# lopunch/CWBNWP-LETKF

Hardware: AMD Instinct MI355X
Metric: analysis grid-points/sec (+ wall-clock per cycle) at k=40, 1/2/4/8 MI355X (higher is better)
Workload: dtype f64

## Files before the change

cwbnwp-letkf_amd/csrc/cwbl_tq40_fill.hip:

```cpp
#include "cwbl_tq40_common.h"

#include <utility>

namespace cwbl {

namespace {

__device__ __forceinline__ void rsum16x2(double &a, double &b) {
  double ab[2] = {a, b};
  rsum16xN(ab);
  a = ab[0];
  b = ab[1];
}

__device__ __forceinline__ void touch(double &x) { asm volatile("" : "+v"(x)); }
__device__ __forceinline__ int touched(int x) {
  asm volatile("" : "+v"(x));
  return x;
}
__device__ __forceinline__ long long touched(long long x) {
  asm volatile("" : "+v"(x));
  return x;
}

template <int KP>
__device__ __forceinline__ void tq40_factor_solve(
    const SolveConsts &c, const SlabDev &slab, Tq40Smem<KP> &sm,
    double (&A)[Tq40Layout<KP>::NS][KP], const long long g0, const bool valid, const int ptot, const int gi, const int q, const int l,
    int2 *__restrict__ info) {
  using LY = Tq40Layout<KP>;
  constexpr int J0 = LY::J0, KT = LY::KT, NS = LY::NS, NV = LY::NV, H = LY::H;
  using SM = Tq40Smem<KP>;
  const int k = c.k;
  const int lp = l < J0 ? l : 0;
  const bool pre = l < J0;
  auto vrow = [&](int vs) { return tq40_vrow<KP>(l, vs); };
  int *const pkeep = reinterpret_cast<int *>(&sm.tq[q][KP][3]);
  *pkeep = ptot;
  const double trace = tq40_trace(sm, q, l, k);

  const double m = (double)c.inflat;
  const double ratio = trace / m - (double)(k - 1);
  int level = 1;
  double dec = 10.0;
  while (level < kQuadLevels && dec < ratio) {
    dec *= 10.0;
    ++level;
  }
  const int R = tq40_wave_rounds(level);
  const int NQ = 8 * R - 1;
  const double2 *qtab = quad_rule(c.quad_r, R, level);
  const int side = l >> 3, n8 = l & 7;
  const double(*T)[4] = sm.tq[q];
  char *const smb = reinterpret_cast<char *>(&sm);
  auto lds = [&](unsigned off) { return *reinterpret_cast<const double *>(smb + off); };
  auto sts = [&](unsigned off, double v) { *reinterpret_cast<double *>(smb + off) = v; };
  const unsigned tq0 = (unsigned)(offsetof(SM, tq) + (size_t)q * sizeof(sm.tq[0])) +
                       (side ? (KP - 1) * 32u : 0u);
  const unsigned dirb = side ? (unsigned)-32 : 32u;
  const unsigned csb = side ? 40u : 8u;
  const unsigned qs0 = (unsigned)(offsetof(SM, qs) + (size_t)q * sizeof(sm.qs[0])) +
                       (side ? (KP - H) * 8u : (H - 1) * 8u);
  const unsigned qz0 = (unsigned)(offsetof(SM, qz) + (size_t)q * sizeof(sm.qz[0]));
  const unsigned bdir = side ? 8u : (unsigned)-8;
  const double sk = sqrt((double)(k - 1));
  auto touch_cols = [&]() {
    sfor<KT - 2>([&](auto jj) {
      constexpr int jl = decltype(jj)::value, J1 = jl + 1, R1 = J1 / 16;
      sfor<NS>([&](auto rr) {
        constexpr int r = decltype(rr)::value;
        if constexpr (16 * r + 15 > J1 || r == R1) touch(A[r][J0 + jl]);
      });
    });
  };

  float *__restrict__ const var = slab.var;
  const int use_rtpp = c.use_rtpp, use_rtps = c.use_rtps;
  const float rtpp_alpha = c.rtpp_alpha, rtps_alpha = c.rtps_alpha;

  float xbl[NV];
  double xb_mean;
  {
    const long long P = tq40_var_index(slab, g0, valid ? gi : 0);
    sfor<NV>([&](auto vv) {
      constexpr int vs = decltype(vv)::value;
      const int i = vrow(vs);
      const bool mem = valid && i < k;
      const float xv = var[P + slab.L * (mem ? i : 0)];
      xbl[vs] = mem ? xv : 0.0f;
    });
    xb_mean = (double)(seq_sum_f32<KP>(xbl) * c.nmember_inv);
  }
  double uxP = pre && l < k ? (double)xbl[0] - xb_mean : 0.0, ux[NS];
  sfor<NS>([&](auto rr) {
    constexpr int r = decltype(rr)::value;
    const int t = J0 + l + 16 * r;
    ux[r] = t < k ? (double)xbl[r + 1] - xb_mean : 0.0;
  });

  touch_cols();
  sfor<J0>([&](auto jj) {
    constexpr int j = decltype(jj)::value, J1 = j + 1;
    const double *pj = sm.pv[q][j];
    const double scal = pj[0], tau = sm.tau[q][j];
    double u2a;
    if constexpr (J1 < J0) u2a = rbcast<J1>(uxP);
    else u2a = rbcast<0>(ux[0]);
    const double xP = (pre && l > J1) ? pj[lp] : 0.0;
    double x[NS], xu = xP * uxP;
    sfor<NS>([&](auto rr) {
      constexpr int r = decltype(rr)::value;
      x[r] = pj[J0 + l + 16 * r];
      xu = fma(x[r], ux[r], xu);
    });
    xu = rsum16(xu);
    const double xsP = xP * scal;
    const double vP = (pre && l == J1) ? 1.0 : xsP;
    const double s2 = fma(scal, xu, u2a);
    uxP = fma(-tau * s2, vP, uxP);
    sfor<NS>([&](auto rr) {
      constexpr int r = decltype(rr)::value;
      const double xs = x[r] * scal;
      double vr;
      if constexpr (J1 == J0 && r == 0) vr = l == 0 ? 1.0 : xs;
      else vr = xs;
      ux[r] = fma(-tau * s2, vr, ux[r]);
    });
  });
  sfor<KT - 2>([&](auto jj) {
    constexpr int jl = decltype(jj)::value, j = J0 + jl;
    constexpr int J1 = jl + 1, R1 = J1 / 16, L1 = J1 % 16;
    const double scal = rbcast<L1>(A[R1][j]), tau = sm.tau[q][j];
    double x[NS], xu = 0.0;
    sfor<NS>([&](auto rr) {
      constexpr int r = decltype(rr)::value;
      if constexpr (16 * r + 15 > J1) {
        const int t = l + 16 * r;
        if constexpr (r == R1) x[r] = t == J1 ? 0.0 : A[r][j];
        else x[r] = A[r][j];
        xu = fma(x[r], ux[r], xu);
      } else {
        x[r] = 0.0;
      }
    });
    xu = rsum16(xu);
    const double s2 = fma(scal, xu, rbcast<L1>(ux[R1]));
    sfor<NS>([&](auto rr) {
      constexpr int r = decltype(rr)::value;
      const int t = l + 16 * r;
      const double xs = x[r] * scal;
      const double vr = t == J1 ? 1.0 : xs;
      ux[r] = fma(-tau * s2, vr, ux[r]);
    });
  });
  if (pre) sm.tq[q][l][3] = uxP;
  sfor<NS>([&](auto rr) {
    constexpr int r = decltype(rr)::value;
    sm.tq[q][J0 + l + 16 * r][3] = ux[r];
  });
  __syncthreads();

  double ys[NV], z[NV];
  sfor<NV>([&](auto vv) { ys[decltype(vv)::value] = 0.0; });
  for (int round = 0; round < R; ++round) {
    const int node = 8 * round + n8;
    const double2 tw = qtab[min(node, NQ - 1)];
    const double sigma = node < NQ ? m * tw.x : 0.0;
    const double omega = node < NQ ? sqrt(m) * tw.y : 1.0;
    double hh[H], mm[H];
    unsigned pw = tq0;
    double dl = lds(pw) + sigma, gt = lds(pw + 24);
    double rdl = rcp64(dl);
    sfor<H - 1>([&](auto tt) {
      constexpr int t = decltype(tt)::value + 1;
      pw += dirb;
      asm volatile("" : "+v"(pw) : "v"(dl));
      const double ct = lds(pw + csb);
      const double lt = ct * rdl;
      hh[t - 1] = gt * rdl;
      mm[t - 1] = lt;
      dl = fma(-lt, ct, lds(pw) + sigma);
      gt = fma(-lt, gt, lds(pw + 24));
      rdl = rcp64(dl);
    });
    const double cm = T[H][1];
    const double dlo = ror8(dl), go = ror8(gt);
    double xv = (gt * dlo - cm * go) / fma(dl, dlo, -cm * cm);
    const bool last = round == R - 1;
    const bool zlane = last && n8 == 7;
    const double om = zlane ? 0.0 : omega;
    unsigned ps = qs0;
    unsigned pz = qz0 + (zlane ? qs0 - (unsigned)offsetof(SM, qs) - (unsigned)q * KP * 8u
                               : KP * 8u);
    const unsigned zdir = zlane ? bdir : 0u;
    auto emit = [&](double x) {
      double s = om * x;
      s += dpp_f64<0xB1>(s);
      s += dpp_f64<0x4E>(s);
      s += dpp_f64<0x141>(s);
      sts(ps, s);
      sts(pz, x);
    };
    emit(xv);
    sfor<H - 1>([&](auto tt) {
      constexpr int t = H - 2 - decltype(tt)::value;
      xv = fma(-mm[t], xv, hh[t]);
      ps += bdir;
      pz += zdir;
      asm volatile("" : "+v"(ps), "+v"(pz) : "v"(xv));
      emit(xv);
    });
    __syncthreads();
    sfor<NV>([&](auto vv) {
      constexpr int vs = decltype(vv)::value;
      const int i = vrow(vs);
      const int ic = i < KP ? i : 0;
      ys[vs] += i < KP ? sm.qs[q][ic] : 0.0;
      if (last) z[vs] = i < KP ? sm.qz[q][ic] : 0.0;
    });
    __syncthreads();
  }
  double dpart = 0.0;
  sfor<NV>([&](auto vv) {
    constexpr int vs = decltype(vv)::value;
    const int i = vrow(vs);
    const double u1 = sm.tq[q][i < KP ? i : 0][2];
    dpart = i < KP ? fma(u1, z[vs], dpart) : dpart;
  });
  const double d = rsum16(dpart);

  double y[NV];
  sfor<NV>([&](auto vv) { y[decltype(vv)::value] = ys[decltype(vv)::value]; });
  touch_cols();
  const int lb = touched(l);
  sfor<KT - 2>([&](auto jj) {
    constexpr int jl = KT - 3 - decltype(jj)::value, j = J0 + jl, J1 = jl + 1;
    constexpr int R1 = J1 / 16, L1 = J1 % 16;
    const double tj = sm.tau[q][j];
    const double scal = rbcast<L1>(A[R1][j]);
    double vv[NS], a = 0.0;
    sfor<NS>([&](auto rr) {
      constexpr int r = decltype(rr)::value;
      if constexpr (16 * r + 15 >= J1) {
        const int t = lb + 16 * r;
        if constexpr (16 * r + 15 > J1) vv[r] = t == J1 ? 1.0 : A[r][j] * scal;
        else vv[r] = t == J1 ? 1.0 : 0.0;
        a = fma(vv[r], y[r + 1], a);
      } else {
        vv[r] = 0.0;
      }
    });
    a = rsum16(a);
    sfor<NS>([&](auto rr) {
      constexpr int r = decltype(rr)::value;
      if constexpr (16 * r + 15 >= J1) y[r + 1] = fma(-tj * a, vv[r], y[r + 1]);
    });
  });
  sfor<J0>([&](auto jj) {
    constexpr int j = J0 - 1 - decltype(jj)::value, J1 = j + 1;
    const double tj = sm.tau[q][j];
    const double *pj = sm.pv[q][j];
    const double scal = pj[0];
    const double v0 = lb == J1 ? 1.0 : (lb < J0 && lb > J1) ? pj[lb] * scal : 0.0;
    double vv[NS];
    double a = v0 * y[0];
    sfor<NS>([&](auto rr) {
      constexpr int r = decltype(rr)::value;
      const double pr = pj[J0 + lb + 16 * r] * scal;
      if constexpr (J1 == J0 && r == 0) vv[r] = lb == 0 ? 1.0 : pr;
      else vv[r] = pr;
      a = fma(vv[r], y[r + 1], a);
    });
    a = rsum16(a);
    y[0] = fma(-tj * a, v0, y[0]);
    sfor<NS>([&](auto rr) {
      constexpr int r = decltype(rr)::value;
      y[r + 1] = fma(-tj * a, vv[r], y[r + 1]);
    });
  });

  float xa[NV];
  sfor<NV>([&](auto vv) {
    constexpr int vs = decltype(vv)::value;
    xa[vs] = vrow(vs) < k ? (float)(xb_mean + (d + sk * y[vs])) : 0.0f;
  });
  if (use_rtpp || use_rtps) {
    const float xa_mean = seq_sum_f32<KP>(xa) * c.nmember_inv;
    double xpl[NV];
    float xap[NV];
    sfor<NV>([&](auto vv) {
      constexpr int vs = decltype(vv)::value;
      const bool mem = vrow(vs) < k;
      xpl[vs] = mem ? (double)xbl[vs] - xb_mean : 0.0;
      xap[vs] = 0.0f;
      if (mem) {
        xap[vs] = xa[vs] - xa_mean;
        if (use_rtpp)
          xap[vs] = (float)((double)((1.0f - rtpp_alpha) * xap[vs]) +
                            (double)rtpp_alpha * xpl[vs]);
      }
    });
    if (use_rtps) {
      double d8 = 0.0;
      sfor<KP>([&](auto mm) {
        constexpr int mb = decltype(mm)::value;
        constexpr int vs = mb < J0 ? 0 : 1 + (mb - J0) / 16, ln = mb < J0 ? mb : (mb - J0) % 16;
        const double xp = rbcast<ln>(xpl[vs]);
        d8 = d8 + xp * xp;
      });
      const float xb_std = (float)d8;
      float sq[NV];
      sfor<NV>([&](auto vv) {
        constexpr int vs = decltype(vv)::value;
        sq[vs] = xap[vs] * xap[vs];
      });
      const float xa_std = seq_sum_f32<KP>(sq);
      const float f = rtps_alpha * sqrtf(xb_std / xa_std) - rtps_alpha + 1.0f;
      sfor<NV>([&](auto vv) { xap[decltype(vv)::value] = xap[decltype(vv)::value] * f; });
    }
    sfor<NV>([&](auto vv) { xa[decltype(vv)::value] = xa_mean + xap[decltype(vv)::value]; });
  }
  const int pt = *pkeep;
  if (valid && pt > 0) {
    const long long P = tq40_var_index(slab, g0, touched(gi));
    sfor<NV>([&](auto vv) {
      constexpr int vs = decltype(vv)::value;
      const int i = vrow(vs);
      if (i < k) var[P + slab.L * i] = xa[vs];
    });
    if (l == 0) info[gi] = make_int2(pt, ratio > dec ? -level : level);
  }
}

}

template <int KP>
__global__ void __launch_bounds__(64, 2)
fill_tq40_factor_kernel(SolveConsts c, SlabDev slab, long long g0, int npts,
                        double *__restrict__ ws, double *__restrict__ aux,
                        int2 *__restrict__ info) {
  using LY = Tq40Layout<KP>;
  using FR = FactorRecord<KP>;
  using FA = FactorAux<KP>;
  constexpr int J0 = LY::J0, KT = LY::KT, NS = LY::NS;
  using SM = Tq40Smem<KP>;
  __shared__ SM sm;

  const int lane = threadIdx.x, q = lane >> 4, l = lane & 15;
  const int g4 = xcd_remap_rev(blockIdx.x, gridDim.x);
  const int gi = 4 * g4 + q;
  const bool valid = gi < npts;
  const int k = c.k;
  const int ptot = valid ? info[gi].x : 0;

  double A[NS][KP];
  double Pb[J0];
  const bool pre = l < J0;
  double ubP, ub[NS];
  tq40_load_record<KP>(ws, g4, q, l, valid, npts, A, Pb, ubP, ub);

  sfor<J0>([&](auto jj) {
    constexpr int j = decltype(jj)::value, J1 = j + 1;
    const double dj = rbcast<j>(Pb[j]);
    double alpha, u1a;
    if constexpr (J1 < J0) {
      alpha = rbcast<J1>(Pb[j]);
      u1a = rbcast<J1>(ubP);
    } else {
      alpha = rbcast<0>(A[0][j]);
      u1a = rbcast<0>(ub[0]);
    }
    const double xP = (pre && l > J1 && l < k) ? Pb[j] : 0.0;
    double x[NS];
    double xx = xP * xP, xb = xP * ubP;
    sfor<NS>([&](auto rr) {
      constexpr int r = decltype(rr)::value;
      const int i = J0 + l + 16 * r;
      x[r] = (i > J1 && i < k) ? A[r][j] : 0.0;
      xx = fma(x[r], x[r], xx);
      xb = fma(x[r], ub[r], xb);
    });
    rsum16x2(xx, xb);
    auto src_of = [&](auto cc, const double &vp, const double (&vs)[NS]) -> const double & {
      constexpr int col = decltype(cc)::value;
      if constexpr (col < J0) return vp;
      else return vs[(col - J0) / 16];
    };
    auto lane_of = [](int col) { return col < J0 ? col : (col - J0) % 16; };
    const Refl h = dlarfg(alpha, xx);
    sm.tq[q][j][0] = dj;
    sm.tq[q][J1][1] = h.beta;
    sm.tau[q][j] = h.tau;
    const double tau = h.tau;
    const double xsP = xP * h.scal;
    double vP = (pre && l == J1) ? 1.0 : xsP;
    double v[NS];
    sm.pv[q][j][(pre && l > 1) ? l : 1] = xP;
    sfor<NS>([&](auto rr) {
      constexpr int r = decltype(rr)::value;
      const double xs = x[r] * h.scal;
      if constexpr (J1 == J0 && r == 0) v[r] = l == 0 ? 1.0 : xs;
      else v[r] = xs;
      sm.pv[q][j][J0 + l + 16 * r] = x[r];
    });
    sm.pv[q][j][0] = h.scal;
    const double s3 = fma(h.scal, xb, u1a);
    ubP = fma(-tau * s3, vP, ubP);
    sfor<NS>([&](auto rr) {
      constexpr int r = decltype(rr)::value;
      ub[r] = fma(-tau * s3, v[r], ub[r]);
    });
    dpp_pin(vP);
    sfor<NS>([&](auto rr) { dpp_pin(v[decltype(rr)::value]); });
    double pa[kNA][NS], pP = 0.0;
    sfor<kNA * NS>([&](auto ii) { pa[decltype(ii)::value / NS][decltype(ii)::value % NS] = 0.0; });
    sfor<KP - J1>([&](auto cc) {
      constexpr int col = J1 + decltype(cc)::value;
      constexpr int LC = lane_of(col);
      const double &vs = src_of(std::integral_constant<int, col>{}, vP, v);
      sfor<NS>([&](auto rr) {
        constexpr int r = decltype(rr)::value;
        constexpr int a = (col - J1) % kNA;
        pa[a][r] = fmac_row<LC>(pa[a][r], vs, A[r][col]);
      });
      if constexpr (col < J0) pP = fmac_row<LC>(pP, vs, Pb[col]);
    });
    if constexpr (J1 < J0) {
      constexpr int NC = J0 - J1, CH = 3;
      sfor<(NC + CH - 1) / CH>([&](auto kk) {
        constexpr int c0 = J1 + CH * decltype(kk)::value;
        constexpr int n = J0 - c0 < CH ? J0 - c0 : CH;
        double cs[n];
        sfor<n>([&](auto cc) {
          constexpr int col = c0 + decltype(cc)::value;
          double s = 0.0;
          sfor<NS>([&](auto rr) {
            constexpr int r = decltype(rr)::value;
            s = fma(A[r][col], v[r], s);
          });
          cs[decltype(cc)::value] = s;
        });
        rsum16xN(cs);
        sfor<n>([&](auto cc) {
          constexpr int col = c0 + decltype(cc)::value;
          pP += l == col ? cs[decltype(cc)::value] : 0.0;
        });
      });
    }
    double pp[NS];
    double sp = vP * pP;
    sfor<NS>([&](auto rr) {
      constexpr int r = decltype(rr)::value;
      pp[r] = acc_sum(pa, r);
      sp = fma(v[r], pp[r], sp);
    });
    const double s1 = tau * rsum16(sp);
    const double wP = fma(-0.5 * tau * s1, vP, tau * pP);
    double wv[NS];
    sfor<NS>([&](auto rr) {
      constexpr int r = decltype(rr)::value;
      wv[r] = fma(-0.5 * tau * s1, v[r], tau * pp[r]);
    });
    double wPp = wP;
    dpp_pin(wPp);
    sfor<NS>([&](auto rr) { dpp_pin(wv[decltype(rr)::value]); });
    sfor<(KP - J1 + kUG - 1) / kUG>([&](auto pp) {
      constexpr int c0 = J1 + kUG * decltype(pp)::value;
      sfor<2>([&](auto hh) {
        constexpr int h = decltype(hh)::value;
        sfor<kUG>([&](auto ee) {
          constexpr int col = c0 + decltype(ee)::value;
          if constexpr (col < KP) {
            constexpr int LC = lane_of(col);
            const double &vs = src_of(std::integral_constant<int, col>{}, vP, v);
            const double &ws = src_of(std::integral_constant<int, col>{}, wPp, wv);
            sfor<NS>([&](auto rr) {
              constexpr int r = decltype(rr)::value;
              if constexpr (h == 0) A[r][col] = fnmac_row<LC>(A[r][col], vs, wv[r]);
              else A[r][col] = fnmac_row<LC>(A[r][col], ws, v[r]);
            });
            if constexpr (col < J0) {
              if constexpr (h == 0) Pb[col] = fnmac_row<LC>(Pb[col], vs, wPp);
              else Pb[col] = fnmac_row<LC>(Pb[col], ws, vP);
            }
          }
        });
      });
    });
  });
  __syncthreads();
  if (pre) sm.tq[q][l][2] = ubP;

  sfor<KT>([&](auto jj) {
    constexpr int jl = decltype(jj)::value, j = J0 + jl;
    constexpr int RJ = jl / 16, LJ = jl % 16;
    const double dj = rbcast<LJ>(A[RJ][j]);
    if constexpr (jl + 2 < KT) {
      constexpr int J1 = jl + 1, R1 = J1 / 16, L1 = J1 % 16;
      const double alpha = rbcast<L1>(A[R1][j]);
      double x[NS], xx = 0.0, xb = 0.0;
      sfor<NS>([&](auto rr) {
        constexpr int r = decltype(rr)::value;
        if constexpr (16 * r + 15 > J1) {
          const int i = J0 + l + 16 * r;
          x[r] = (i > j + 1 && i < k) ? A[r][j] : 0.0;
          xx = fma(x[r], x[r], xx);
          xb = fma(x[r], ub[r], xb);
        } else {
          x[r] = 0.0;
        }
      });
      rsum16x2(xx, xb);
      const Refl h = dlarfg(alpha, xx);
      const double tau = h.tau;
      sm.tq[q][j][0] = dj;
      sm.tq[q][j + 1][1] = h.beta;
      sm.tau[q][j] = tau;
      double v[NS];
      sfor<NS>([&](auto rr) {
        constexpr int r = decltype(rr)::value;
        const int t = l + 16 * r;
        const double xs = x[r] * h.scal;
        v[r] = t == J1 ? 1.0 : xs;
        if constexpr (r == R1) A[r][j] = t == J1 ? h.scal : x[r];
        else if constexpr (16 * r + 15 > J1) A[r][j] = x[r];
      });
      const double s3 = fma(h.scal, xb, rbcast<L1>(ub[R1]));
      sfor<NS>([&](auto rr) {
        constexpr int r = decltype(rr)::value;
        ub[r] = fma(-tau * s3, v[r], ub[r]);
      });
      double pa[kNA][NS];
      sfor<kNA * NS>([&](auto ii) { pa[decltype(ii)::value / NS][decltype(ii)::value % NS] = 0.0; });
      sfor<NS>([&](auto rr) { dpp_pin(v[decltype(rr)::value]); });
      sfor<KT - J1>([&](auto cc) {
        constexpr int cl = J1 + decltype(cc)::value;
        sfor<NS>([&](auto rr) {
          constexpr int r = decltype(rr)::value;
          if constexpr (16 * r + 15 > jl) {
            constexpr int a = (cl - J1) % kNA;
            pa[a][r] = fmac_row<cl % 16>(pa[a][r], v[cl / 16], A[r][J0 + cl]);
          }
        });
      });
      double pp[NS], sp = 0.0;
      sfor<NS>([&](auto rr) {
        constexpr int r = decltype(rr)::value;
        pp[r] = acc_sum(pa, r);
        if constexpr (16 * r + 15 > jl) sp = fma(v[r], pp[r], sp);
      });
      const double s1 = tau * rsum16(sp);
      double wv[NS];
      sfor<NS>([&](auto rr) {
        constexpr int r = decltype(rr)::value;
        wv[r] = fma(-0.5 * tau * s1, v[r], tau * pp[r]);
      });
      sfor<NS>([&](auto rr) { dpp_pin(wv[decltype(rr)::value]); });
      sfor<(KT - J1 + kUG - 1) / kUG>([&](auto pp) {
        constexpr int c0 = J1 + kUG * decltype(pp)::value;
        sfor<2>([&](auto hh) {
          constexpr int h = decltype(hh)::value;
          sfor<kUG>([&](auto ee) {
            constexpr int cl = c0 + decltype(ee)::value;
            if constexpr (cl < KT) {
              sfor<NS>([&](auto rr) {
                constexpr int r = decltype(rr)::value;
                if constexpr (16 * r + 15 > jl) {
                  if constexpr (h == 0)
                    A[r][J0 + cl] = fnmac_row<cl % 16>(A[r][J0 + cl], v[cl / 16], wv[r]);
                  else
                    A[r][J0 + cl] = fnmac_row<cl % 16>(A[r][J0 + cl], wv[cl / 16], v[r]);
                }
              });
            }
          });
        });
      });
    } else {
      const double ej = rbcast<LJ>(A[RJ][j - 1]);
      sm.tq[q][j][0] = dj;
      if constexpr (jl == KT - 1) sm.tq[q][j][1] = ej;
    }
  });
  sfor<NS>([&](auto rr) {
    constexpr int r = decltype(rr)::value;
    const int i = J0 + l + 16 * r;
    sm.tq[q][i][2] = ub[r];
  });
  if (l == 0) {
    sm.tq[q][0][1] = 0.0;
    sm.tq[q][KP][1] = 0.0;
  }
  __syncthreads();

  if (valid) {
    const unsigned wb = (unsigned)gi * (unsigned)FR::WORDS;
    auto st = [&](unsigned w, double x) { gst(ws, 8u * (wb + w), x); };
    sfor<(KP + 15) / 16>([&](auto rr) {
      constexpr int r = decltype(rr)::value;
      const int i = l + 16 * r;
      if (16 * r + 15 < KP || i < KP) st((unsigned)(FR::D + i), sm.tq[q][i][0]);
    });
    if (pre) st((unsigned)(FR::U1 + l), ubP);
    sfor<NS>([&](auto rr) {
      constexpr int r = decltype(rr)::value;
      st((unsigned)(FR::U1 + J0 + l + 16 * r), ub[r]);
    });
    sfor<J0>([&](auto jj) {
      constexpr int j = decltype(jj)::value, J1 = j + 1;
      const double *pj = sm.pv[q][j];
      if (pre && l >= J1) st((unsigned)(FR::col(j) + l - J1), pj[l == J1 ? 0 : l]);
      sfor<NS>([&](auto rr) {
        constexpr int r = decltype(rr)::value;
        const int i = J0 + l + 16 * r;
        if constexpr (J1 == J0 && r == 0) st((unsigned)(FR::col(j) + i - J1), pj[l == 0 ? 0 : i]);
        else st((unsigned)(FR::col(j) + i - J1), pj[i]);
      });
    });
    sfor<KT - 2>([&](auto jj) {
      constexpr int jl = decltype(jj)::value, j = J0 + jl, J1 = jl + 1;
      sfor<NS>([&](auto rr) {
        constexpr int r = decltype(rr)::value;
        if constexpr (16 * r + 15 >= J1) {
          const int t = l + 16 * r;
          if (t >= J1) st((unsigned)(FR::col(j) + t - J1), A[r][j]);
        }
      });
    });
    if (l == 0) st((unsigned)FR::EL, 0.0);
    const unsigned ab = (unsigned)gi * (unsigned)FA::WORDS;
    sfor<(KP + 15) / 16>([&](auto rr) {
      constexpr int r = decltype(rr)::value;
      const int i = l + 16 * r;
      if (16 * r + 15 < KP || i < KP) {
        gst(aux, 8u * (ab + (unsigned)(FA::B + i)), sm.tq[q][i][1]);
        const double tj = sm.tau[q][i < KP - 2 ? i : 0];
        gst(aux, 8u * (ab + (unsigned)(FA::T + i)), i < KP - 2 ? tj : 0.0);
      }
    });
  }

  tq40_factor_solve<KP>(c, slab, sm, A, g0, valid, ptot, gi, q, l, info);
}

template <int KP>
__global__ void __launch_bounds__(64, 2)
solve_tq40_factor_kernel(SolveConsts c, SlabDev slab, long long g0, int npts,
                         const double *__restrict__ ws, const double *__restrict__ aux,
                         int2 *__restrict__ info) {
  using LY = Tq40Layout<KP>;
  using FR = FactorRecord<KP>;
  using FA = FactorAux<KP>;
  constexpr int J0 = LY::J0, KT = LY::KT, NS = LY::NS;
  using SM = Tq40Smem<KP>;
  __shared__ SM sm;

  const int lane = threadIdx.x, q = lane >> 4, l = lane & 15;
  const int g4 = xcd_remap_rev(blockIdx.x, gridDim.x);
  const int gi = 4 * g4 + q;
  const bool valid = gi < npts;
  const int ptot = valid ? info[gi].x : 0;
  const bool pre = l < J0;

  const __amdgpu_buffer_rsrc_t rs = rec_rsrc(ws + (size_t)(4 * g4) * FR::WORDS, 4 * FR::WORDS);
  const unsigned rq = (unsigned)(valid ? q : npts - 4 * g4) * (unsigned)FR::WORDS;
  auto rw = [&](unsigned vword, unsigned cword) {
    const unsigned cb = 8u * cword;
    const auto v = __builtin_amdgcn_raw_buffer_load_b64(rs, (int)(8u * vword + (cb & 4095u)),
                                                        (int)(cb & ~4095u), 0);
    return __longlong_as_double(((long long)v[1] << 32) | (unsigned)v[0]);
  };
  auto rwb = [&](unsigned vbyte, unsigned cword) {
    const unsigned cb = 8u * cword;
    const auto v = __builtin_amdgcn_raw_buffer_load_b64(rs, (int)(vbyte + (cb & 4095u)),
                                                        (int)(cb & ~4095u), 0);
    return __longlong_as_double(((long long)v[1] << 32) | (unsigned)v[0]);
  };
  const unsigned rl = rq + (unsigned)l;
  double A[NS][KP];
  double c1P[J0], c1[J0][NS];
  sfor<J0>([&](auto jj) {
    constexpr int j = decltype(jj)::value, J1 = j + 1;
    c1P[j] = rw(rq + (unsigned)((pre && l > J1) ? l - J1 : 0), (unsigned)FR::col(j));
    sfor<NS>([&](auto rr) {
      constexpr int r = decltype(rr)::value;
      if constexpr (J1 == J0 && r == 0)
        c1[j][r] = rwb(rec_off(l != 0, (int)rl), (unsigned)(FR::col(j) + J0 + 16 * r - J1));
      else
        c1[j][r] = rw(rl, (unsigned)(FR::col(j) + J0 + 16 * r - J1));
    });
  });
  sfor<KT - 2>([&](auto jj) {
    constexpr int jl = decltype(jj)::value, j = J0 + jl, J1 = jl + 1;
    sfor<NS>([&](auto rr) {
      constexpr int r = decltype(rr)::value;
      if constexpr (16 * r >= J1) {
        A[r][j] = rw(rl, (unsigned)(FR::col(j) + 16 * r - J1));
      } else if constexpr (16 * r + 15 >= J1) {
        const int t = l + 16 * r;
        A[r][j] = rwb(rec_off(t >= J1, (int)rq + t - J1), (unsigned)FR::col(j));
      }
    });
  });
  double dg[(KP + 15) / 16];
  sfor<(KP + 15) / 16>([&](auto rr) {
    constexpr int r = decltype(rr)::value;
    const int i = l + 16 * r;
    dg[r] = rw(rq + (unsigned)(i < KP ? i : 0), (unsigned)FR::D);
  });
  double ubP, ub[NS];
  {
    const double b = rw(rq + (unsigned)(pre ? l : 0), (unsigned)FR::U1);
    ubP = pre ? b : 0.0;
  }
  sfor<NS>([&](auto rr) {
    constexpr int r = decltype(rr)::value;
    ub[r] = rw(rl, (unsigned)(FR::U1 + J0 + 16 * r));
  });
  const __amdgpu_buffer_rsrc_t ra = rec_rsrc(aux + (size_t)(4 * g4) * FA::WORDS, 4 * FA::WORDS);
  const unsigned aq = (unsigned)(valid ? q : npts - 4 * g4) * (unsigned)FA::WORDS;
  constexpr int NA = (KP + 15) / 16;
  static_assert(16 * (NA - 1) + 8 == KP, "the last run of an aux half is half a row");
  const int l2 = l < 8 ? l + 16 * (NA - 1) : l + 16 * (NA - 2);
  auto arow = [&](int r) { return r < NA - 1 ? l + 16 * r : l2; };
  double bt[NA], ta[NA];
  sfor<NA>([&](auto rr) {
    constexpr int r = decltype(rr)::value;
    const unsigned off = 8u * (aq + (unsigned)arow(r));
    const auto vb = __builtin_amdgcn_raw_buffer_load_b64(ra, (int)(off + 8u * FA::B), 0, 0);
    const auto vt = __builtin_amdgcn_raw_buffer_load_b64(ra, (int)(off + 8u * FA::T), 0, 0);
    bt[r] = __longlong_as_double(((long long)vb[1] << 32) | (unsigned)vb[0]);
    ta[r] = __longlong_as_double(((long long)vt[1] << 32) | (unsigned)vt[0]);
  });

  sfor<(KP + 15) / 16>([&](auto rr) {
    constexpr int r = decltype(rr)::value;
    const int i = l + 16 * r;
    sm.tq[q][i < KP ? i : KP][0] = dg[r];
  });
  sm.tq[q][pre ? l : KP][2] = ubP;
  sfor<NS>([&](auto rr) {
    constexpr int r = decltype(rr)::value;
    sm.tq[q][J0 + l + 16 * r][2] = ub[r];
  });
  sfor<NA>([&](auto rr) {
    constexpr int r = decltype(rr)::value;
    sm.tq[q][arow(r)][1] = bt[r];
    sm.tau[q][arow(r)] = ta[r];
  });
  sm.tq[q][KP][1] = 0.0;

  sfor<J0>([&](auto jj) {
    constexpr int j = decltype(jj)::value, J1 = j + 1;
    sm.pv[q][j][(pre && l > J1) ? l : 0] = c1P[j];
    sfor<NS>([&](auto rr) {
      constexpr int r = decltype(rr)::value;
      sm.pv[q][j][J0 + l + 16 * r] = c1[j][r];
    });
  });
  __syncthreads();

  tq40_factor_solve<KP>(c, slab, sm, A, g0, valid, ptot, gi, q, l, info);
}

hipError_t launch_fill_tq40_factor(hipStream_t s, int kp, SolveConsts c, SlabDev slab,
                                   long long g0, int npts, double *ws, double *aux, int2 *info) {
  if (npts <= 0) return hipSuccess;
  if (c.quad_r == nullptr || aux == nullptr || kp != kTq4KP) return hipErrorInvalidValue;
  const dim3 grid((npts + 3) / 4);
  hipLaunchKernelGGL((fill_tq40_factor_kernel<kTq4KP>), grid, dim3(64), 0, s, c, slab, g0, npts,
                     ws, aux, info);
  return hipGetLastError();
}

hipError_t launch_solve_tq40_factor(hipStream_t s, int kp, SolveConsts c, SlabDev slab,
                                    long long g0, int npts, const double *ws, const double *aux,
                                    int2 *info) {
  if (npts <= 0) return hipSuccess;
  if (c.quad_r == nullptr || aux == nullptr || kp != kTq4KP) return hipErrorInvalidValue;
  const dim3 grid((npts + 3) / 4);
  hipLaunchKernelGGL((solve_tq40_factor_kernel<kTq4KP>), grid, dim3(64), 0, s, c, slab, g0, npts,
                     ws, aux, info);
  return hipGetLastError();
}

}
```

Measured before the change: 417.2 million.

## Prefetch background state, quadrature nodes and LDS rows ahead in TQ40 solve

Hoists the background-ensemble loads out of the factor solve so the solve kernel can issue them earlier, interleaved with the factor reloads. An AHEAD template variant prefetches the next quadrature node and the next tridiagonal row from LDS one step early, and it reorders when the register columns are touched. The RTPS spread is now computed from squares taken once per lane and reduced via DPP row ops. These changes aim to hide global and LDS latency, at the cost of higher register pressure that may lower occupancy.

```diff
diff --git a/cwbnwp-letkf_amd/csrc/cwbl_tq40_fill.hip b/cwbnwp-letkf_amd/csrc/cwbl_tq40_fill.hip
--- a/cwbnwp-letkf_amd/csrc/cwbl_tq40_fill.hip
+++ b/cwbnwp-letkf_amd/csrc/cwbl_tq40_fill.hip
@@ -24,9 +24,23 @@
 }
 
 template <int KP>
+__device__ __forceinline__ void tq40_load_xb(const SlabDev &slab, const long long g0,
+                                             const bool valid, const int gi, const int l,
+                                             const int k, float (&xv)[Tq40Layout<KP>::NV]) {
+  const float *__restrict__ const var = slab.var;
+  const long long P = tq40_var_index(slab, g0, valid ? gi : 0);
+  sfor<Tq40Layout<KP>::NV>([&](auto vv) {
+    constexpr int vs = decltype(vv)::value;
+    const int i = tq40_vrow<KP>(l, vs);
+    xv[vs] = var[P + slab.L * ((valid && i < k) ? i : 0)];
+  });
+}
+
+template <int KP, bool AHEAD>
 __device__ __forceinline__ void tq40_factor_solve(
     const SolveConsts &c, const SlabDev &slab, Tq40Smem<KP> &sm,
-    double (&A)[Tq40Layout<KP>::NS][KP], const long long g0, const bool valid, const int ptot, const int gi, const int q, const int l,
+    double (&A)[Tq40Layout<KP>::NS][KP], const float (&xbv)[Tq40Layout<KP>::NV], const long long g0,
+    const bool valid, const int ptot, const int gi, const int q, const int l,
     int2 *__restrict__ info) {
   using LY = Tq40Layout<KP>;
   constexpr int J0 = LY::J0, KT = LY::KT, NS = LY::NS, NV = LY::NV, H = LY::H;
@@ -50,6 +64,8 @@
   const int R = tq40_wave_rounds(level);
   const int NQ = 8 * R - 1;
   const double2 *qtab = quad_rule(c.quad_r, R, level);
+  double2 twn;
+  if constexpr (AHEAD) twn = qtab[min(l & 7, NQ - 1)];
   const int side = l >> 3, n8 = l & 7;
   const double(*T)[4] = sm.tq[q];
   char *const smb = reinterpret_cast<char *>(&sm);
@@ -81,13 +97,10 @@
   float xbl[NV];
   double xb_mean;
   {
-    const long long P = tq40_var_index(slab, g0, valid ? gi : 0);
     sfor<NV>([&](auto vv) {
       constexpr int vs = decltype(vv)::value;
-      const int i = vrow(vs);
-      const bool mem = valid && i < k;
-      const float xv = var[P + slab.L * (mem ? i : 0)];
-      xbl[vs] = mem ? xv : 0.0f;
+      const bool mem = valid && vrow(vs) < k;
+      xbl[vs] = mem ? xbv[vs] : 0.0f;
     });
     xb_mean = (double)(seq_sum_f32<KP>(xbl) * c.nmember_inv);
   }
@@ -98,7 +111,6 @@
     ux[r] = t < k ? (double)xbl[r + 1] - xb_mean : 0.0;
   });
 
-  touch_cols();
   sfor<J0>([&](auto jj) {
     constexpr int j = decltype(jj)::value, J1 = j + 1;
     const double *pj = sm.pv[q][j];
@@ -130,6 +142,10 @@
   sfor<KT - 2>([&](auto jj) {
     constexpr int jl = decltype(jj)::value, j = J0 + jl;
     constexpr int J1 = jl + 1, R1 = J1 / 16, L1 = J1 % 16;
+    sfor<NS>([&](auto rr) {
+      constexpr int r = decltype(rr)::value;
+      if constexpr (16 * r + 15 > J1 || r == R1) touch(A[r][j]);
+    });
     const double scal = rbcast<L1>(A[R1][j]), tau = sm.tau[q][j];
     double x[NS], xu = 0.0;
     sfor<NS>([&](auto rr) {
@@ -164,24 +180,43 @@
   sfor<NV>([&](auto vv) { ys[decltype(vv)::value] = 0.0; });
   for (int round = 0; round < R; ++round) {
     const int node = 8 * round + n8;
-    const double2 tw = qtab[min(node, NQ - 1)];
+    double2 tw;
+    if constexpr (AHEAD) {
+      tw = twn;
+      if (round + 1 < R) twn = qtab[min(node + 8, NQ - 1)];
+    } else {
+      tw = qtab[min(node, NQ - 1)];
+    }
     const double sigma = node < NQ ? m * tw.x : 0.0;
     const double omega = node < NQ ? sqrt(m) * tw.y : 1.0;
     double hh[H], mm[H];
     unsigned pw = tq0;
     double dl = lds(pw) + sigma, gt = lds(pw + 24);
-    double rdl = rcp64(dl);
+    double nd, nc, ng;
+    auto next_row = [&]() {
+      pw += dirb;
+      nd = lds(pw);
+      nc = lds(pw + csb);
+      ng = lds(pw + 24);
+    };
+    if constexpr (AHEAD) next_row();
     sfor<H - 1>([&](auto tt) {
       constexpr int t = decltype(tt)::value + 1;
-      pw += dirb;
-      asm volatile("" : "+v"(pw) : "v"(dl));
-      const double ct = lds(pw + csb);
+      if constexpr (!AHEAD) {
+        asm volatile("" : "+v"(pw) : "v"(dl));
+        next_row();
+      }
+      const double dt = nd, ct = nc, g = ng;
+      if constexpr (AHEAD && t < H - 1) {
+        asm volatile("" : "+v"(pw) : "v"(dl));
+        next_row();
+      }
+      const double rdl = rcp64(dl);
       const double lt = ct * rdl;
       hh[t - 1] = gt * rdl;
       mm[t - 1] = lt;
-      dl = fma(-lt, ct, lds(pw) + sigma);
-      gt = fma(-lt, gt, lds(pw + 24));
-      rdl = rcp64(dl);
+      dl = fma(-lt, ct, dt + sigma);
+      gt = fma(-lt, gt, g);
     });
     const double cm = T[H][1];
     const double dlo = ror8(dl), go = ror8(gt);
@@ -301,12 +336,16 @@
       }
     });
     if (use_rtps) {
-      double d8 = 0.0;
+      double d8 = 0.0, sq8[NV];
+      sfor<NV>([&](auto vv) {
+        constexpr int vs = decltype(vv)::value;
+        sq8[vs] = xpl[vs] * xpl[vs];
+        dpp_pin(sq8[vs]);
+      });
       sfor<KP>([&](auto mm) {
         constexpr int mb = decltype(mm)::value;
         constexpr int vs = mb < J0 ? 0 : 1 + (mb - J0) / 16, ln = mb < J0 ? mb : (mb - J0) % 16;
-        const double xp = rbcast<ln>(xpl[vs]);
-        d8 = d8 + xp * xp;
+        d8 = fmac_row<ln>(d8, sq8[vs], 1.0);
       });
       const float xb_std = (float)d8;
       float sq[NV];
@@ -640,7 +679,9 @@
     });
   }
 
-  tq40_factor_solve<KP>(c, slab, sm, A, g0, valid, ptot, gi, q, l, info);
+  float xv[LY::NV];
+  tq40_load_xb<KP>(slab, g0, valid, gi, l, k, xv);
+  tq40_factor_solve<KP, false>(c, slab, sm, A, xv, g0, valid, ptot, gi, q, l, info);
 }
 
 template <int KP>
@@ -677,31 +718,6 @@
     return __longlong_as_double(((long long)v[1] << 32) | (unsigned)v[0]);
   };
   const unsigned rl = rq + (unsigned)l;
-  double A[NS][KP];
-  double c1P[J0], c1[J0][NS];
-  sfor<J0>([&](auto jj) {
-    constexpr int j = decltype(jj)::value, J1 = j + 1;
-    c1P[j] = rw(rq + (unsigned)((pre && l > J1) ? l - J1 : 0), (unsigned)FR::col(j));
-    sfor<NS>([&](auto rr) {
-      constexpr int r = decltype(rr)::value;
-      if constexpr (J1 == J0 && r == 0)
-        c1[j][r] = rwb(rec_off(l != 0, (int)rl), (unsigned)(FR::col(j) + J0 + 16 * r - J1));
-      else
-        c1[j][r] = rw(rl, (unsigned)(FR::col(j) + J0 + 16 * r - J1));
-    });
-  });
-  sfor<KT - 2>([&](auto jj) {
-    constexpr int jl = decltype(jj)::value, j = J0 + jl, J1 = jl + 1;
-    sfor<NS>([&](auto rr) {
-      constexpr int r = decltype(rr)::value;
-      if constexpr (16 * r >= J1) {
-        A[r][j] = rw(rl, (unsigned)(FR::col(j) + 16 * r - J1));
-      } else if constexpr (16 * r + 15 >= J1) {
-        const int t = l + 16 * r;
-        A[r][j] = rwb(rec_off(t >= J1, (int)rq + t - J1), (unsigned)FR::col(j));
-      }
-    });
-  });
   double dg[(KP + 15) / 16];
   sfor<(KP + 15) / 16>([&](auto rr) {
     constexpr int r = decltype(rr)::value;
@@ -732,6 +748,33 @@
     bt[r] = __longlong_as_double(((long long)vb[1] << 32) | (unsigned)vb[0]);
     ta[r] = __longlong_as_double(((long long)vt[1] << 32) | (unsigned)vt[0]);
   });
+  double A[NS][KP];
+  double c1P[J0], c1[J0][NS];
+  sfor<J0>([&](auto jj) {
+    constexpr int j = decltype(jj)::value, J1 = j + 1;
+    c1P[j] = rw(rq + (unsigned)((pre && l > J1) ? l - J1 : 0), (unsigned)FR::col(j));
+    sfor<NS>([&](auto rr) {
+      constexpr int r = decltype(rr)::value;
+      if constexpr (J1 == J0 && r == 0)
+        c1[j][r] = rwb(rec_off(l != 0, (int)rl), (unsigned)(FR::col(j) + J0 + 16 * r - J1));
+      else
+        c1[j][r] = rw(rl, (unsigned)(FR::col(j) + J0 + 16 * r - J1));
+    });
+  });
+  float xv[LY::NV];
+  tq40_load_xb<KP>(slab, g0, valid, gi, l, c.k, xv);
+  sfor<KT - 2>([&](auto jj) {
+    constexpr int jl = decltype(jj)::value, j = J0 + jl, J1 = jl + 1;
+    sfor<NS>([&](auto rr) {
+      constexpr int r = decltype(rr)::value;
+      if constexpr (16 * r >= J1) {
+        A[r][j] = rw(rl, (unsigned)(FR::col(j) + 16 * r - J1));
+      } else if constexpr (16 * r + 15 >= J1) {
+        const int t = l + 16 * r;
+        A[r][j] = rwb(rec_off(t >= J1, (int)rq + t - J1), (unsigned)FR::col(j));
+      }
+    });
+  });
 
   sfor<(KP + 15) / 16>([&](auto rr) {
     constexpr int r = decltype(rr)::value;
@@ -760,7 +803,7 @@
   });
   __syncthreads();
 
-  tq40_factor_solve<KP>(c, slab, sm, A, g0, valid, ptot, gi, q, l, info);
+  tq40_factor_solve<KP, true>(c, slab, sm, A, xv, g0, valid, ptot, gi, q, l, info);
 }
 
 hipError_t launch_fill_tq40_factor(hipStream_t s, int kp, SolveConsts c, SlabDev slab,
```

Result: faster. 437.3 million, median of 6 (+4.8%).
